# gmum/3d-point-clouds-autocomplete

Measured on AMD Instinct MI355X. Metric: train-step point-clouds/sec at B=64, N=2048 (Chamfer+EMD), higher is better.
Workload: dtype f32 storage / accumulation / results; matrix products formed from f16 x2 (bf16 x3) pieces of the fp32 operands — NOT IEEE-fp32 products: the all-fp32-kernel step is `value_strict_fp32`

## Files before the change

3d-point-clouds-autocomplete_amd/csrc/emd.hip:

```cpp
#include "hp_common.h"
#include <algorithm>
#include <map>
#include <mutex>
#include <vector>


namespace {

#ifndef HP_EMD_PARTS
#define HP_EMD_PARTS 4
#endif
constexpr int kThreads = 64 * HP_EMD_PARTS;
constexpr int kLevels = 9;
constexpr int kStage = 8;
constexpr int kSpare = 8;
constexpr float kLog2e = 1.4426950408889634f;

typedef float f32x16 __attribute__((ext_vector_type(16)));
typedef float f32x8 __attribute__((ext_vector_type(8)));
typedef float f2 __attribute__((ext_vector_type(2)));

#define HP_SLOAD16(dst, ptr, off) asm volatile("s_load_dwordx16 %0, %1, " #off : "=s"(dst) : "s"(ptr) : "memory")
#define HP_SLOAD8(dst, ptr, off) asm volatile("s_load_dwordx8 %0, %1, " #off : "=s"(dst) : "s"(ptr) : "memory")
#define HP_PIN() __builtin_amdgcn_sched_barrier(0)

__host__ __device__ constexpr float level_l2e(int lev) {
    return (lev == 0 ? -16384.f : lev == 1 ? -4096.f : lev == 2 ? -1024.f : lev == 3 ? -256.f : lev == 4 ? -64.f
            : lev == 5 ? -16.f : lev == 6 ? -4.f : lev == 7 ? -1.f : -0.25f) * kLog2e;
}
__host__ __device__ constexpr float underflow_r2(int lev) { return 152.f / -level_l2e(lev); }

constexpr int kParts = HP_EMD_PARTS;
constexpr int kRowsPerWg = kThreads / kParts;
inline int pad_up(int x) { return (x + 2 * kStage * kParts - 1) / (2 * kStage * kParts) * (2 * kStage * kParts); }

struct WsLayout {
    int NP, MP;
    long plp, prp, rr, flp, frp, permL, permR, blkL, blkR, tileL, tileR, flag, per_cloud;
};
constexpr int kBlk = 8;
constexpr int kTile = 64;
inline WsLayout ws_layout(int n, int m) {
    WsLayout w;
    w.NP = pad_up(n);
    w.MP = pad_up(m);
    w.plp = 0;
    w.prp = w.plp + (long)(w.NP + kSpare) * 4;
    w.rr = w.prp + (long)(w.MP + kSpare) * 4;
    w.flp = w.rr + (long)(w.MP + kSpare);
    w.frp = w.flp + (long)(w.NP + kSpare) * 16;
    w.permL = w.frp + (long)(w.MP + kSpare) * 16;
    w.permR = w.permL + w.NP;
    w.blkL = w.permR + w.MP;
    w.blkR = w.blkL + 6L * (w.NP / kBlk);
    w.tileL = w.blkR + 6L * (w.MP / kBlk);
    w.tileR = w.tileL + 6L * (w.NP / kTile);
    w.flag = w.tileR + 6L * (w.MP / kTile);
    w.per_cloud = w.flag + 16;
    return w;
}

std::mutex g_s2_mu;
std::map<int, hipStream_t> g_s2_streams;
constexpr int kMaxChains = 4;
constexpr int kOrderMaxLog = 12;
hp::Switch g_chains("HP_EMD_CHAINS", 2, 1, kMaxChains);
hp::Switch g_cull("HP_EMD_CULL", 3, 0, kLevels);
hp::Switch g_final_derive("HP_EMD_FINAL_DERIVE", 1);
hp::Switch g_rows1("HP_EMD_ROWS1_R", 0, 0, 4), g_rows2("HP_EMD_ROWS2_R", 0, 0, 4), g_grad2("HP_EMD_GRAD2_R", 0, 0, 2);
struct EmdSwitches {
    int chains, cull, rows1, rows2, grad2;
    bool derive;
};
EmdSwitches read_switches() {
    return {g_chains.get(), g_cull.get(), g_rows1.get(), g_rows2.get(), g_grad2.get(), g_final_derive.get() != 0};
}

struct Ctx {
    int n, m, NP, MP;
    const float* xyz1;
    const float* xyz2;
    float* temp;
    float* ws;
    int plp, prp, rr, flp, frp, permL, permR, blkL, blkR, tileL, tileR, flag;
    long per_cloud;
    float acc_scale = 0.f;
};
inline Ctx make_ctx(int n, int m, const float* xyz1, const float* xyz2, float* temp, float* ws) {
    const WsLayout L = ws_layout(n, m);
    Ctx c;
    c.n = n; c.m = m; c.NP = L.NP; c.MP = L.MP;
    c.xyz1 = xyz1; c.xyz2 = xyz2; c.temp = temp; c.ws = ws;
    c.plp = (int)L.plp; c.prp = (int)L.prp; c.rr = (int)L.rr; c.flp = (int)L.flp; c.frp = (int)L.frp;
    c.permL = (int)L.permL; c.permR = (int)L.permR; c.blkL = (int)L.blkL; c.blkR = (int)L.blkR; c.tileL = (int)L.tileL; c.tileR = (int)L.tileR;
    c.flag = (int)L.flag; c.per_cloud = L.per_cloud;
    c.acc_scale = 0.f;
    return c;
}

__device__ __forceinline__ long pair8(int i, int comp) { return (long)(i >> 1) * 8 + comp * 2 + (i & 1); }
__device__ __forceinline__ long pair32(int i, int comp) { return (long)(i >> 1) * 32 + comp * 2 + (i & 1); }

__global__ __launch_bounds__(256) void emd_init_kernel(Ctx c, float multiL, float multiR) {
    const int cloud = blockIdx.y;
    float* ws = c.ws + (long)cloud * c.per_cloud;
    float* remL = c.temp + (long)cloud * (c.n + c.m) * 2;
    float* remR = remL + c.n;
    const float* P = c.xyz1 + (long)cloud * c.n * 3;
    const float* Q = c.xyz2 + (long)cloud * c.m * 3;
    const int NPp = (c.NP + kSpare) / 2, MPp = (c.MP + kSpare) / 2;
    if (blockIdx.x == 0 && threadIdx.x == 0) ws[c.flag] = 0.f;
    for (int i = blockIdx.x * 256 + threadIdx.x; i < NPp + MPp; i += gridDim.x * 256) {
        const bool left = i < NPp;
        const int pr = left ? i : i - NPp, j0 = 2 * pr, j1 = j0 + 1;
        const int cnt = left ? c.n : c.m;
        const float* src = left ? P : Q;
        const bool ok0 = j0 < cnt, ok1 = j1 < cnt;
        const float x0 = ok0 ? src[j0 * 3] : 0.f, y0 = ok0 ? src[j0 * 3 + 1] : 0.f, z0 = ok0 ? src[j0 * 3 + 2] : 0.f;
        const float x1 = ok1 ? src[j1 * 3] : 0.f, y1 = ok1 ? src[j1 * 3 + 1] : 0.f, z1 = ok1 ? src[j1 * 3 + 2] : 0.f;
        float4* p8 = reinterpret_cast<float4*>(ws + (left ? c.plp : c.prp) + (long)pr * 8);
        float4* p32 = reinterpret_cast<float4*>(ws + (left ? c.flp : c.frp) + (long)pr * 32);
        const float4 a = make_float4(x0, x1, y0, y1), b = make_float4(z0, z1, 0.f, 0.f), zero = make_float4(0.f, 0.f, 0.f, 0.f);
        p8[0] = a;
        p8[1] = b;
        p32[0] = a;
        p32[1] = b;
#pragma unroll
        for (int q = 2; q < 8; ++q) p32[q] = zero;
        if (left) {
            if (ok0) remL[j0] = multiL;
            if (ok1) remL[j1] = multiL;
        } else {
            *reinterpret_cast<float2*>(ws + c.rr + j0) = make_float2(ok0 ? multiR : 0.f, ok1 ? multiR : 0.f);
            if (ok0) remR[j0] = multiR;
            if (ok1) remR[j1] = multiR;
        }
    }
}

// ... 176 lines not shown
    }
    const int NB = NPx / kBlk, NT = NPx / kTile;
    float* bb = ws + (left ? c.blkL : c.blkR);
    float* lb = box0;
    for (int g = tid; g < NB; g += kOrderThreads) {
        float lo[3] = {kFar, kFar, kFar}, hi[3] = {-kFar, -kFar, -kFar};
        for (int j = g * kBlk; j < min(g * kBlk + kBlk, cnt); ++j) {
            const uint32_t i = key[j] & imask;
            lo[0] = fminf(lo[0], X[i]); hi[0] = fmaxf(hi[0], X[i]);
            lo[1] = fminf(lo[1], Y[i]); hi[1] = fmaxf(hi[1], Y[i]);
            lo[2] = fminf(lo[2], Z[i]); hi[2] = fmaxf(hi[2], Z[i]);
        }
#pragma unroll
        for (int q = 0; q < 3; ++q) {
            bb[q * NB + g] = lo[q];
            bb[(3 + q) * NB + g] = hi[q];
            lb[g * 6 + q] = lo[q];
            lb[g * 6 + 3 + q] = hi[q];
        }
    }
    __syncthreads();
    float* tb = ws + (left ? c.tileL : c.tileR);
    for (int t = tid; t < NT; t += kOrderThreads) {
        float lo[3] = {kFar, kFar, kFar}, hi[3] = {-kFar, -kFar, -kFar};
        for (int g = t * (kTile / kBlk); g < (t + 1) * (kTile / kBlk); ++g) {
#pragma unroll
            for (int q = 0; q < 3; ++q) {
                lo[q] = fminf(lo[q], lb[g * 6 + q]);
                hi[q] = fmaxf(hi[q], lb[g * 6 + 3 + q]);
            }
        }
#pragma unroll
        for (int q = 0; q < 3; ++q) {
            tb[q * NT + t] = lo[q];
            tb[(3 + q) * NT + t] = hi[q];
        }
    }
    if (left && tid == 0) {
        ws[c.flag] = 1.f;
        ws[c.flag + 1] = cull > 1 ? underflow_r2(1) : 3.0e38f;
        ws[c.flag + 2] = cull > 2 ? underflow_r2(2) : 3.0e38f;
    }
}

#define PAIRC(lo, hi, u, c) \
    ((u) < 2 ? f2{(lo)[(u)*8 + (c)*2], (lo)[(u)*8 + (c)*2 + 1]} : f2{(hi)[((u)-2) * 8 + (c)*2], (hi)[((u)-2) * 8 + (c)*2 + 1]})

__device__ __forceinline__ f2 splat(float v) { return f2{v, v}; }
__device__ __forceinline__ f2 sqdist2(f2 dx, f2 dy, f2 dz) {
    return __builtin_elementwise_fma(dz, dz, __builtin_elementwise_fma(dy, dy, dx * dx));
}
__device__ __forceinline__ f2 exp2_2(f2 a) { return f2{__builtin_amdgcn_exp2f(a.x), __builtin_amdgcn_exp2f(a.y)}; }

template <bool DO3, bool DO1, int R>
__global__ __launch_bounds__(kThreads) void emd_rows1_kernel(Ctx c, int lev1, float l2e3, float l2e1) {
    __shared__ float part3[kParts][kRowsPerWg * R], part1[kParts][kRowsPerWg * R];
    const int cloud = blockIdx.y;
    const int lrow = threadIdx.x % kRowsPerWg;
    const int part = __builtin_amdgcn_readfirstlane(threadIdx.x / kRowsPerWg);
    float* ws = c.ws + (long)cloud * c.per_cloud;
    float* remL = c.temp + (long)cloud * (c.n + c.m) * 2;
    float* ratioL = remL + c.n + c.m;
    int k[R];
    bool ok[R];
    f2 px2[R], py2[R], pz2[R], rl2[R], acc3[R], acc1[R];
#pragma unroll
    for (int r = 0; r < R; ++r) {
        k[r] = (blockIdx.x * R + r) * kRowsPerWg + lrow;
        ok[r] = k[r] < c.n;
        float px = 0.f, py = 0.f, pz = 0.f, rl = 0.f;
        if (ok[r]) {
            px = ws[c.plp + pair8(k[r], 0)];
            py = ws[c.plp + pair8(k[r], 1)];
            pz = ws[c.plp + pair8(k[r], 2)];
            if (DO3) rl = ratioL[k[r]];
        }
        px2[r] = splat(px);
        py2[r] = splat(py);
        pz2[r] = splat(pz);
        rl2[r] = splat(rl);
        acc3[r] = splat(0.f);
        acc1[r] = f2{part == 0 ? 1e-9f : 0.f, 0.f};
    }
    const f2 l3 = splat(l2e3), l1 = splat(l2e1);
    const int cand = c.MP / kParts;
    const float* p = ws + c.prp + (long)part * cand * 4;
    const float* q = ws + c.rr + (long)part * cand;
    f32x16 a0, a1, b0, b1;
    f32x8 w0 = {}, w1 = {};
    auto work = [&](const f32x16& lo, const f32x16& hi, const f32x8& w) {
#pragma unroll
        for (int u = 0; u < kStage / 2; ++u) {
#pragma unroll
            for (int r = 0; r < R; ++r) {
                const f2 d = sqdist2(PAIRC(lo, hi, u, 0) - px2[r], PAIRC(lo, hi, u, 1) - py2[r], PAIRC(lo, hi, u, 2) - pz2[r]);
                if (DO3) {
                    acc3[r] = __builtin_elementwise_fma(exp2_2(l3 * d) * rl2[r], PAIRC(lo, hi, u, 3), acc3[r]);
                }
                if (DO1) {
                    acc1[r] = __builtin_elementwise_fma(exp2_2(l1 * d), f2{w[u * 2], w[u * 2 + 1]}, acc1[r]);
                }
            }
        }
    };
    HP_SLOAD16(a0, p, 0x0);
    HP_SLOAD16(a1, p, 0x40);
    if (DO1) HP_SLOAD8(w0, q, 0x0);
    asm volatile("s_waitcnt lgkmcnt(0)" : "+s"(a0), "+s"(a1), "+s"(w0));
    for (int l0 = 0; l0 < cand; l0 += 2 * kStage) {
        p += kStage * 4;
        q += kStage;
        HP_SLOAD16(b0, p, 0x0);
        HP_SLOAD16(b1, p, 0x40);
        if (DO1) HP_SLOAD8(w1, q, 0x0);
        HP_PIN();
        work(a0, a1, w0);
        asm volatile("s_waitcnt lgkmcnt(0)" : "+s"(b0), "+s"(b1), "+s"(w1), "+v"(acc3[0]), "+v"(acc1[0]), "+v"(acc3[R - 1]), "+v"(acc1[R - 1]));
        p += kStage * 4;
        q += kStage;
        HP_SLOAD16(a0, p, 0x0);
        HP_SLOAD16(a1, p, 0x40);
        if (DO1) HP_SLOAD8(w0, q, 0x0);
        HP_PIN();
        work(b0, b1, w1);
        asm volatile("s_waitcnt lgkmcnt(0)" : "+s"(a0), "+s"(a1), "+s"(w0), "+v"(acc3[0]), "+v"(acc1[0]), "+v"(acc3[R - 1]), "+v"(acc1[R - 1]));
    }
    float s3[R], s1[R];
#pragma unroll
    for (int r = 0; r < R; ++r) {
        s3[r] = acc3[r].x + acc3[r].y;
        s1[r] = acc1[r].x + acc1[r].y;
        part3[part][r * kRowsPerWg + lrow] = s3[r];
        part1[part][r * kRowsPerWg + lrow] = s1[r];
    }
    __syncthreads();
    if (part != 0) return;
#pragma unroll
    for (int r = 0; r < R; ++r) {
        if (!ok[r]) continue;
        float t3 = s3[r], t1 = s1[r];
#pragma unroll
        for (int q2 = 1; q2 < kParts; ++q2) {
            t3 += part3[q2][r * kRowsPerWg + lrow];
            t1 += part1[q2][r * kRowsPerWg + lrow];
        }
        float rem = remL[k[r]];
        if (DO3) {
            rem = fmaxf(0.0f, rem - t3);
            remL[k[r]] = rem;
        }
        if (DO1) {
            const float v = rem / t1;
            ratioL[k[r]] = v;
            ws[c.plp + pair8(k[r], 3)] = v;
            ws[c.flp + pair32(k[r], 3 + lev1)] = v;
        }
    }
}

template <int R>
__global__ __launch_bounds__(kThreads) void emd_rows2_kernel(Ctx c, int lev, float l2e) {
    __shared__ float parts[kParts][kRowsPerWg * R];
    const int cloud = blockIdx.y;
    const int lrow = threadIdx.x % kRowsPerWg;
    const int part = __builtin_amdgcn_readfirstlane(threadIdx.x / kRowsPerWg);
    float* ws = c.ws + (long)cloud * c.per_cloud;
    float* remR = c.temp + (long)cloud * (c.n + c.m) * 2 + c.n;
    float* ratioR = remR + c.m + c.n;
    int l[R];
    bool ok[R];
    f2 qx2[R], qy2[R], qz2[R], acc2[R];
#pragma unroll
    for (int r = 0; r < R; ++r) {
        l[r] = (blockIdx.x * R + r) * kRowsPerWg + lrow;
        ok[r] = l[r] < c.m;
        float qx = 0.f, qy = 0.f, qz = 0.f;
        if (ok[r]) {
            qx = ws[c.prp + pair8(l[r], 0)];
            qy = ws[c.prp + pair8(l[r], 1)];
            qz = ws[c.prp + pair8(l[r], 2)];
        }
        qx2[r] = splat(qx);
        qy2[r] = splat(qy);
        qz2[r] = splat(qz);
        acc2[r] = splat(0.f);
    }
    const f2 lv = splat(l2e);
    const int cand = c.NP / kParts;
    const float* p = ws + c.plp + (long)part * cand * 4;
    f32x16 a0, a1, b0, b1;
    auto work = [&](const f32x16& lo, const f32x16& hi) {
#pragma unroll
        for (int u = 0; u < kStage / 2; ++u) {
#pragma unroll
            for (int r = 0; r < R; ++r) {
                const f2 d = sqdist2(qx2[r] - PAIRC(lo, hi, u, 0), qy2[r] - PAIRC(lo, hi, u, 1), qz2[r] - PAIRC(lo, hi, u, 2));
                acc2[r] = __builtin_elementwise_fma(exp2_2(lv * d), PAIRC(lo, hi, u, 3), acc2[r]);
            }
        }
    };
    HP_SLOAD16(a0, p, 0x0);
    HP_SLOAD16(a1, p, 0x40);
    asm volatile("s_waitcnt lgkmcnt(0)" : "+s"(a0), "+s"(a1));
    for (int k0 = 0; k0 < cand; k0 += 2 * kStage) {
        p += kStage * 4;
        HP_SLOAD16(b0, p, 0x0);
        HP_SLOAD16(b1, p, 0x40);
        HP_PIN();
        work(a0, a1);
        if (R == 1) asm volatile("s_waitcnt lgkmcnt(0)" : "+s"(b0), "+s"(b1), "+v"(acc2[0]));
        else asm volatile("s_waitcnt lgkmcnt(0)" : "+s"(b0), "+s"(b1), "+v"(acc2[0]), "+v"(acc2[R - 1]));
        p += kStage * 4;
        HP_SLOAD16(a0, p, 0x0);
        HP_SLOAD16(a1, p, 0x40);
        HP_PIN();
        work(b0, b1);
        if (R == 1) asm volatile("s_waitcnt lgkmcnt(0)" : "+s"(a0), "+s"(a1), "+v"(acc2[0]));
        else asm volatile("s_waitcnt lgkmcnt(0)" : "+s"(a0), "+s"(a1), "+v"(acc2[0]), "+v"(acc2[R - 1]));
    }
    float acc[R];
#pragma unroll
    for (int r = 0; r < R; ++r) {
        acc[r] = acc2[r].x + acc2[r].y;
        parts[part][r * kRowsPerWg + lrow] = acc[r];
    }
    __syncthreads();
    if (part != 0) return;
#pragma unroll
    for (int r = 0; r < R; ++r) {
        if (!ok[r]) continue;
        float a = acc[r];
#pragma unroll
        for (int q2 = 1; q2 < kParts; ++q2) a += parts[q2][r * kRowsPerWg + lrow];
        const float rr = remR[l[r]];
        const float sumr = a * rr;
        const float consumption = fminf(rr / (sumr + 1e-9f), 1.0f);
        const float v = consumption * rr;
        const float rem = fmaxf(0.0f, rr - sumr);
        ratioR[l[r]] = v;
        remR[l[r]] = rem;
        ws[c.prp + pair8(l[r], 3)] = v;
        ws[c.rr + l[r]] = rem;
        ws[c.frp + pair32(l[r], 3 + lev)] = v;
    }
}

__device__ __forceinline__ float box_gap2(const float (&tlo)[3], const float (&thi)[3], float cx0, float cy0, float cz0, float cx1, float cy1,
                                          float cz1) {
    const float gx = fmaxf(0.f, fmaxf(cx0 - thi[0], tlo[0] - cx1));
    const float gy = fmaxf(0.f, fmaxf(cy0 - thi[1], tlo[1] - cy1));
    const float gz = fmaxf(0.f, fmaxf(cz0 - thi[2], tlo[2] - cz1));
    return gx * gx + gy * gy + gz * gz;
}
__device__ __forceinline__ void load_tile_box(const float* tb, int NT, int t, float (&lo)[3], float (&hi)[3]) {
#pragma unroll
    for (int q = 0; q < 3; ++q) {
        lo[q] = t < NT ? tb[q * NT + t] : kFar;
        hi[q] = t < NT ? tb[(3 + q) * NT + t] : -kFar;
    }
}

template <bool DO3, bool DO1, int R, int P>
__global__ __launch_bounds__(64 * P) void emd_rows1_cull_kernel(Ctx c, int lev1, float l2e3, float l2e1, float thr3, float thr1) {
    __shared__ float part3[P][kRowsPerWg * R], part1[P][kRowsPerWg * R];
    const int cloud = blockIdx.y;
    const int lrow = threadIdx.x % kRowsPerWg;
    const int part = __builtin_amdgcn_readfirstlane(threadIdx.x / kRowsPerWg);
    float* ws = c.ws + (long)cloud * c.per_cloud;
    float* remL = c.temp + (long)cloud * (c.n + c.m) * 2;
    float* ratioL = remL + c.n + c.m;
    int k[R];
    bool ok[R];
    f2 px2[R], py2[R], pz2[R], rl2[R], acc3[R], acc1[R];
    float tlo[R][3], thi[R][3];
#pragma unroll
    for (int r = 0; r < R; ++r) {
        k[r] = (blockIdx.x * R + r) * kRowsPerWg + lrow;
        ok[r] = k[r] < c.n;
        float px = 0.f, py = 0.f, pz = 0.f, rl = 0.f;
        if (ok[r]) {
            px = ws[c.plp + pair8(k[r], 0)];
            py = ws[c.plp + pair8(k[r], 1)];
            pz = ws[c.plp + pair8(k[r], 2)];
            if (DO3) rl = ratioL[k[r]];
        }
        px2[r] = splat(px);
        py2[r] = splat(py);
        pz2[r] = splat(pz);
        rl2[r] = splat(rl);
        acc3[r] = splat(0.f);
        acc1[r] = f2{part == 0 ? 1e-9f : 0.f, 0.f};
        load_tile_box(ws + c.tileL, c.NP / kTile, blockIdx.x * R + r, tlo[r], thi[r]);
    }
    const f2 l3 = splat(l2e3), l1 = splat(l2e1);
    const int NB = c.MP / kBlk, nblk = (NB + P - 1) / P;
    const float* bb = ws + c.blkR;
    const float* prec = ws + c.prp;
// ... 522 lines not shown
        parts[part][3][r * kRowsPerWg + lrow] = cost[r];
    }
    __syncthreads();
    float total = 0.f;
    if (part == 0) {
#pragma unroll
        for (int r = 0; r < R; ++r) {
#pragma unroll
            for (int q2 = 1; q2 < kParts; ++q2) {
                sx[r] += parts[q2][0][r * kRowsPerWg + lrow];
                sy[r] += parts[q2][1][r * kRowsPerWg + lrow];
                sz[r] += parts[q2][2][r * kRowsPerWg + lrow];
                cost[r] += parts[q2][3][r * kRowsPerWg + lrow];
            }
            if (ok[r]) {
                const int lo = ws[c.flag] != 0.f ? reinterpret_cast<const int*>(ws + c.permR)[l[r]] : l[r];
                float* g = grad2 + ((long)cloud * c.m + lo) * 3;
                if (c.acc_scale != 0.f) {
                    g[0] = __builtin_fmaf(c.acc_scale, sx[r], g[0]);
                    g[1] = __builtin_fmaf(c.acc_scale, sy[r], g[1]);
                    g[2] = __builtin_fmaf(c.acc_scale, sz[r], g[2]);
                } else {
                    g[0] = sx[r];
                    g[1] = sy[r];
                    g[2] = sz[r];
                }
                total += cost[r];
            }
        }
    }
    if (WITH_COST) {
        const float t = hp::block_sum(total, red);
        if (threadIdx.x == 0) partials[(long)cloud * gridDim.x + blockIdx.x] = t;
    }
}

__global__ __launch_bounds__(256) void emd_cost_finish_kernel(const float* __restrict__ partials, int per_cloud, float* __restrict__ out) {
    __shared__ double red[4];
    const float* p = partials + (long)blockIdx.x * per_cloud;
    double s = 0;
    for (int i = threadIdx.x; i < per_cloud; i += 256) s += (double)p[i];
    const double t = hp::block_sum(s, red);
    if (threadIdx.x == 0) out[blockIdx.x] = (float)t;
}

struct LevelChain {
    Ctx c;
    int b;
    hipStream_t stream;
    bool final_remainL;
    float multiL, multiR;
    int rows1_r, rows2_r;
    int cull;
    int logpL = 0, logpR = 0;
    dim3 ginit, g1[3], g2[3];

    static int log2_ceil64(int x) {
        int l = 6;
        while ((1 << l) < x) ++l;
        return l;
    }
    float radius2(int lev) const { return lev < cull ? underflow_r2(lev) : 3.0e38f; }

    LevelChain(int b_, int n, int m, const float* xyz1, const float* xyz2, float* temp, float* ws, hipStream_t st, bool frl,
               const EmdSwitches& sw)
        : b(b_), stream(st), final_remainL(frl), cull(sw.cull) {
        const WsLayout L = ws_layout(n, m);
        c = make_ctx(n, m, xyz1, xyz2, temp, ws);
        if (n >= m) {
            multiL = 1;
            multiR = (float)(n / m);
        } else {
            multiL = (float)(m / n);
            multiR = 1;
        }
        logpL = log2_ceil64(n);
        logpR = log2_ceil64(m);
        if (logpL > kOrderMaxLog || logpR > kOrderMaxLog) cull = 0;
        for (int i = 0; i < 3; ++i) {
            const int r = 1 << i;
            g1[i] = dim3((n + r * kRowsPerWg - 1) / (r * kRowsPerWg), b);
            g2[i] = dim3((m + r * kRowsPerWg - 1) / (r * kRowsPerWg), b);
        }
        ginit = dim3(((L.NP + L.MP + 2 * kSpare) / 2 + 255) / 256, b);
        auto pick = [&](int rows, int cap) {
            for (int r = cap; r > 1; r >>= 1)
                if ((long)b * ((rows + r * kRowsPerWg - 1) / (r * kRowsPerWg)) * (kThreads / 64) >= 2048) return r;
            return 1;
        };
        rows1_r = sw.rows1 ? sw.rows1 : pick(n, 2);
        rows2_r = sw.rows2 ? sw.rows2 : pick(m, 4);
    }

    template <bool D3, bool D1>
    void rows1(int lev3, int lev1) const {
        const float l2e3 = D3 ? level_l2e(lev3) : 0.f, l2e1 = D1 ? level_l2e(lev1) : 0.f;
        const int i = rows1_r == 4 ? 2 : rows1_r == 2 ? 1 : 0;
        const int clev = D1 ? lev1 : lev3;
        if (cull > 0 && clev < cull) {
            const float t3 = D3 ? radius2(lev3) : 0.f, t1 = D1 ? radius2(lev1) : 0.f;
            hipLaunchKernelGGL((emd_rows1_cull_kernel<D3, D1, 1, kParts>), g1[0], dim3(kThreads), 0, stream, c, lev1, l2e3, l2e1, t3, t1);
            return;
        }
        if (rows1_r == 4) hipLaunchKernelGGL((emd_rows1_kernel<D3, D1, 4>), g1[i], dim3(kThreads), 0, stream, c, lev1, l2e3, l2e1);
        else if (rows1_r == 2) hipLaunchKernelGGL((emd_rows1_kernel<D3, D1, 2>), g1[i], dim3(kThreads), 0, stream, c, lev1, l2e3, l2e1);
        else hipLaunchKernelGGL((emd_rows1_kernel<D3, D1, 1>), g1[i], dim3(kThreads), 0, stream, c, lev1, l2e3, l2e1);
    }
    void rows2(int lev) const {
        const int i = rows2_r == 4 ? 2 : rows2_r == 2 ? 1 : 0;
        if (cull > 0 && lev < cull) {
            const float t = radius2(lev);
            hipLaunchKernelGGL((emd_rows2_cull_kernel<1, kParts>), g2[0], dim3(kThreads), 0, stream, c, lev, level_l2e(lev), t);
            return;
        }
        if (rows2_r == 4) hipLaunchKernelGGL(emd_rows2_kernel<4>, g2[i], dim3(kThreads), 0, stream, c, lev, level_l2e(lev));
        else if (rows2_r == 2) hipLaunchKernelGGL(emd_rows2_kernel<2>, g2[i], dim3(kThreads), 0, stream, c, lev, level_l2e(lev));
        else hipLaunchKernelGGL(emd_rows2_kernel<1>, g2[i], dim3(kThreads), 0, stream, c, lev, level_l2e(lev));
    }
    static constexpr int kSteps = 2 + 2 * kLevels;
    void step(int s) const {
        if (s == 0) {
            if (cull > 0) {
                const int lp = std::max(logpL, logpR);
                const size_t lds = ((size_t)18 << lp) + kCells * 4;
                if (lds > 48 * 1024)
                    (void)hipFuncSetAttribute(reinterpret_cast<const void*>(emd_order_kernel), hipFuncAttributeMaxDynamicSharedMemorySize, (int)lds);
                hipLaunchKernelGGL(emd_order_kernel, dim3(2, b), dim3(kOrderThreads), lds, stream, c, multiL, multiR, logpL, logpR, cull);
            } else {
                hipLaunchKernelGGL(emd_init_kernel, ginit, dim3(256), 0, stream, c, multiL, multiR);
            }
        } else if (s == 1) {
            rows1<false, true>(0, 0);
        } else {
            const int lev = (s - 2) >> 1;
            if (((s - 2) & 1) == 0) rows2(lev);
            else if (lev + 1 < kLevels) rows1<true, true>(lev, lev + 1);
            else if (final_remainL) rows1<true, false>(lev, lev);
        }
    }
};

int run_levels(int b, int n, int m, const float* xyz1, const float* xyz2, float* temp, float* ws, Ctx* out, hipStream_t stream,
               bool final_remainL, const EmdSwitches& sw) {
    const LevelChain ch(b, n, m, xyz1, xyz2, temp, ws, stream, final_remainL, sw);
    for (int s = 0; s < LevelChain::kSteps; ++s) ch.step(s);
    *out = ch.c;
    return (int)hipGetLastError();
}

constexpr int kPlainTile = 1024;

__global__ __launch_bounds__(kThreads) void emd_plain_init_kernel(int n, int m, float* __restrict__ temp, float multiL, float multiR) {
    float* remL = temp + (long)blockIdx.y * (n + m) * 2;
    for (int i = blockIdx.x * kThreads + threadIdx.x; i < n + m; i += gridDim.x * kThreads) remL[i] = i < n ? multiL : multiR;
}

template <int PHASE>
__global__ __launch_bounds__(kThreads) void emd_plain_kernel(int n, int m, const float* __restrict__ xyz1, const float* __restrict__ xyz2,
                                                             float* __restrict__ temp, float* __restrict__ match, float l2e, int first) {
    __shared__ float4 tile[kPlainTile];
    const int cloud = blockIdx.y, tid = threadIdx.x;
    float* remL = temp + (long)cloud * (n + m) * 2;
    float* remR = remL + n;
    float* ratioL = remR + m;
    float* ratioR = ratioL + n;
    constexpr bool kRowsL = PHASE != 2;
    const int rows = kRowsL ? n : m, cands = kRowsL ? m : n;
    const float* R = (kRowsL ? xyz1 : xyz2) + (long)cloud * rows * 3;
    const float* C = (kRowsL ? xyz2 : xyz1) + (long)cloud * cands * 3;
    const float* cw = PHASE == 1 ? remR : PHASE == 2 ? ratioL : ratioR;
    const int row = blockIdx.x * kThreads + tid;
    const bool ok = row < rows;
    float rx = 0.f, ry = 0.f, rz = 0.f, rl = 0.f;
    if (ok) {
        rx = R[row * 3];
        ry = R[row * 3 + 1];
        rz = R[row * 3 + 2];
        if (PHASE == 3) rl = ratioL[row];
    }
    float sum = PHASE == 1 ? 1e-9f : 0.f;
    float* mcol = match + (long)cloud * m * n + row;
    for (int c0 = 0; c0 < cands; c0 += kPlainTile) {
        const int cnt = min(kPlainTile, cands - c0);
        for (int t = tid; t < cnt; t += kThreads) {
            const float* s = C + (long)(c0 + t) * 3;
            tile[t] = make_float4(s[0], s[1], s[2], cw[c0 + t]);
        }
        __syncthreads();
        if (ok) {
#pragma unroll 4
            for (int t = 0; t < cnt; ++t) {
                const float4 c = tile[t];
                const float d = kRowsL ? hp::sqdist(c.x - rx, c.y - ry, c.z - rz) : hp::sqdist(rx - c.x, ry - c.y, rz - c.z);
                const float e = __builtin_amdgcn_exp2f(l2e * d);
                if (PHASE == 3) {
                    const float er = e * rl;
                    float* mp = mcol + (long)(c0 + t) * n;
                    *mp = first ? er * c.w : __builtin_fmaf(er, c.w, *mp);
                    sum = __builtin_fmaf(er, c.w, sum);
                } else {
                    sum = __builtin_fmaf(e, c.w, sum);
                }
            }
        }
        __syncthreads();
    }
    if (!ok) return;
    if (PHASE == 1) {
        ratioL[row] = remL[row] / sum;
    } else if (PHASE == 2) {
        const float rr = remR[row];
        const float sumr = sum * rr;
        const float consumption = fminf(rr / (sumr + 1e-9f), 1.0f);
        ratioR[row] = consumption * rr;
        remR[row] = fmaxf(0.0f, rr - sumr);
    } else {
        remL[row] = fmaxf(0.0f, remL[row] - sum);
    }
}

}

HP_API int hp_emd_set_rows_per_lane(int rows1, int rows2, int grad2) {
    auto okv = [](int v, bool four) { return v == 0 || v == 1 || v == 2 || (four && v == 4); };
    HP_CHECK_ARG(okv(rows1, true) && okv(rows2, true) && okv(grad2, false));
    g_rows1.set(rows1);
    g_rows2.set(rows2);
    g_grad2.set(grad2);
    return 0;
}

HP_API int hp_emd_set_final_derive(int on) { return g_final_derive.set(on); }

HP_API int hp_emd_set_cull(int levels) {
    HP_CHECK_ARG(levels >= -1 && levels <= kLevels);
    return g_cull.set(levels);
}

HP_API int hp_emd_set_chains(int chains) {
    HP_CHECK_ARG(chains == -1 || (chains >= 1 && chains <= kMaxChains));
    return g_chains.set(chains);
}

HP_API int hp_approxmatch(int b, int n, int m, const float* xyz1, const float* xyz2, float* match, float* temp, hipStream_t stream) {
    HP_CHECK_ARG(b >= 0 && n > 0 && m > 0);
    if (b == 0) return 0;
    HP_CHECK_ARG(xyz1 && xyz2 && match && temp && b <= 65535);
    float multiL, multiR;
    if (n >= m) {
        multiL = 1;
        multiR = (float)(n / m);
    } else {
        multiL = (float)(m / n);
        multiR = 1;
    }
    const dim3 blk(kThreads), gL((n + kThreads - 1) / kThreads, b), gR((m + kThreads - 1) / kThreads, b);
    hipLaunchKernelGGL(emd_plain_init_kernel, dim3((n + m + kThreads - 1) / kThreads, b), blk, 0, stream, n, m, temp, multiL, multiR);
    for (int lev = 0; lev < kLevels; ++lev) {
        const float l2e = level_l2e(lev);
        hipLaunchKernelGGL(emd_plain_kernel<1>, gL, blk, 0, stream, n, m, xyz1, xyz2, temp, match, l2e, 0);
        hipLaunchKernelGGL(emd_plain_kernel<2>, gR, blk, 0, stream, n, m, xyz1, xyz2, temp, match, l2e, 0);
        hipLaunchKernelGGL(emd_plain_kernel<3>, gL, blk, 0, stream, n, m, xyz1, xyz2, temp, match, l2e, lev == 0);
    }
    HP_RETURN_LAST_ERROR();
}

HP_API long hp_approxmatch_workspace_floats(int b, int n, int m) { return (long)b * ws_layout(n, m).per_cloud; }

HP_API int hp_approxmatch_ws(int b, int n, int m, const float* xyz1, const float* xyz2, float* match, float* temp, float* ws,
                             hipStream_t stream) {
    HP_CHECK_ARG(b >= 0 && n > 0 && m > 0);
    if (b == 0) return 0;
    HP_CHECK_ARG(xyz1 && xyz2 && match && temp && ws && b <= 65535);
    Ctx c;
    EmdSwitches sw = read_switches();
    sw.cull = 0;
    int rc = run_levels(b, n, m, xyz1, xyz2, temp, ws, &c, stream, true, sw);
    if (rc) return rc;
    hipLaunchKernelGGL(emd_match_kernel, dim3((n + kThreads - 1) / kThreads, (m + kLT - 1) / kLT, b), dim3(kThreads), 0, stream, c,
                       match);
    HP_RETURN_LAST_ERROR();
}

HP_API long hp_emd_partials_floats(int b, int n, int m) { return (long)b * ((std::max(n, m) + kRowsPerWg - 1) / kRowsPerWg); }

namespace {
int emd_forward_impl(int b, int n, int m, const float* xyz1, const float* xyz2, float* temp, float* ws, float* partials,
                     float* cost, float* grad1, float* grad2, float acc_scale, hipStream_t stream, hipStream_t after);
}
HP_API int hp_emd_forward(int b, int n, int m, const float* xyz1, const float* xyz2, float* temp, float* ws, float* partials,
                          float* cost, float* grad1, float* grad2, hipStream_t stream) {
    return emd_forward_impl(b, n, m, xyz1, xyz2, temp, ws, partials, cost, grad1, grad2, 0.f, stream, nullptr);
}

HP_API int hp_emd_forward_acc(int b, int n, int m, const float* xyz1, const float* xyz2, float* temp, float* ws, float* partials,
                              float* cost, float* grad2_acc, float scale, hipStream_t stream, hipStream_t after) {
    HP_CHECK_ARG(grad2_acc && scale != 0.f);
    return emd_forward_impl(b, n, m, xyz1, xyz2, temp, ws, partials, cost, nullptr, grad2_acc, scale, stream, after);
}

namespace {
template <bool WITH_COST>
int launch_grad2(const Ctx& c, int b, float* grad2, float* partials, int rows, bool derive, hipStream_t stream) {
    const int mbr = (c.m + 2 * kRowsPerWg - 1) / (2 * kRowsPerWg);
    const bool two = (rows ? rows : ((long)b * mbr * (kThreads / 64) >= 2048 ? 2 : 1)) == 2;
    const dim3 grid(two ? mbr : (c.m + kRowsPerWg - 1) / kRowsPerWg, b);
    if (two) {
        if (derive) hipLaunchKernelGGL((emd_grad2_kernel<WITH_COST, 2, true>), grid, dim3(kThreads), 0, stream, c, grad2, partials);
        else hipLaunchKernelGGL((emd_grad2_kernel<WITH_COST, 2, false>), grid, dim3(kThreads), 0, stream, c, grad2, partials);
    } else {
        if (derive) hipLaunchKernelGGL((emd_grad2_kernel<WITH_COST, 1, true>), grid, dim3(kThreads), 0, stream, c, grad2, partials);
        else hipLaunchKernelGGL((emd_grad2_kernel<WITH_COST, 1, false>), grid, dim3(kThreads), 0, stream, c, grad2, partials);
    }
    return (int)grid.x;
}

int emd_final_sweep(Ctx c, int b, float* partials, float* cost, float* grad1, float* grad2, float acc_scale, hipStream_t stream,
                    hipStream_t after, const EmdSwitches& sw) {
    const int n = c.n;
    int rc = 0;
    c.acc_scale = acc_scale;
    if (after && after != stream) {
        rc = hp_order_streams(after, stream);
        if (rc) return rc;
    }
    const int nb = (n + kRowsPerWg - 1) / kRowsPerWg;
    if (grad2) {
        const int gb = launch_grad2<true>(c, b, grad2, partials, sw.grad2, sw.derive, stream);
        hipLaunchKernelGGL(emd_cost_finish_kernel, dim3(b), dim3(256), 0, stream, partials, gb, cost);
        if (grad1) {
            if (sw.derive) hipLaunchKernelGGL(emd_cost_grad1_kernel<true>, dim3(nb, b), dim3(kThreads), 0, stream, c, partials, grad1);
            else hipLaunchKernelGGL(emd_cost_grad1_kernel<false>, dim3(nb, b), dim3(kThreads), 0, stream, c, partials, grad1);
        }
    } else {
        if (sw.derive) hipLaunchKernelGGL(emd_cost_grad1_kernel<true>, dim3(nb, b), dim3(kThreads), 0, stream, c, partials, grad1);
        else hipLaunchKernelGGL(emd_cost_grad1_kernel<false>, dim3(nb, b), dim3(kThreads), 0, stream, c, partials, grad1);
        hipLaunchKernelGGL(emd_cost_finish_kernel, dim3(b), dim3(256), 0, stream, partials, nb, cost);
    }
    HP_RETURN_LAST_ERROR();
}


hipStream_t chain_stream(hipStream_t stream, int i) {
    int cur = 0, dev = 0;
    if (hipGetDevice(&cur) != hipSuccess) return nullptr;
    dev = cur;
    if (stream && hipStreamGetDevice(stream, &dev) != hipSuccess) {
        (void)hipGetLastError();
        dev = cur;
    }
    std::lock_guard<std::mutex> lock(g_s2_mu);
    auto it = g_s2_streams.find(dev * kMaxChains + i);
    if (it != g_s2_streams.end()) return it->second;
    hipStream_t s = nullptr;
    if (dev == cur || hipSetDevice(dev) == hipSuccess) {
        int lo = 0, hi = 0;
        (void)hipDeviceGetStreamPriorityRange(&lo, &hi);
        if (hipStreamCreateWithPriority(&s, hipStreamNonBlocking, hi) != hipSuccess) {
            (void)hipGetLastError();
            s = nullptr;
        }
        if (dev != cur) (void)hipSetDevice(cur);
    } else {
        (void)hipGetLastError();
    }
    g_s2_streams[dev * kMaxChains + i] = s;
    return s;
}

int emd_forward_impl(int b, int n, int m, const float* xyz1, const float* xyz2, float* temp, float* ws, float* partials,
                     float* cost, float* grad1, float* grad2, float acc_scale, hipStream_t stream, hipStream_t after) {
    HP_CHECK_ARG(b >= 0 && n > 0 && m > 0);
    if (b == 0) return 0;
    HP_CHECK_ARG(xyz1 && xyz2 && temp && ws && partials && cost && b <= 65535);
    const EmdSwitches sw = read_switches();
    hipStreamCaptureStatus cap = hipStreamCaptureStatusNone;
    (void)hipStreamIsCapturing(stream, &cap);
    int nch = cap == hipStreamCaptureStatusNone ? sw.chains : 1;
    while (nch > 1 && (long)(b / nch) * ((std::min(n, m) + kRowsPerWg - 1) / kRowsPerWg) * (kThreads / 64) < 2048) --nch;
    hipStream_t st[kMaxChains] = {stream};
    for (int i = 1; i < nch; ++i) {
        st[i] = chain_stream(stream, i);
        if (!st[i]) nch = 1;
    }
    if (nch <= 1) {
        Ctx c;
        const int rc = run_levels(b, n, m, xyz1, xyz2, temp, ws, &c, stream, false, sw);
        return rc ? rc : emd_final_sweep(c, b, partials, cost, grad1, grad2, acc_scale, stream, after, sw);
    }
    const WsLayout L = ws_layout(n, m);
    int rc = 0;
    for (int i = 1; i < nch && !rc; ++i) rc = hp_order_streams(stream, st[i]);
    if (rc) return rc;
    std::vector<LevelChain> ch;
    ch.reserve(nch);
    for (int i = 0; i < nch; ++i) {
        const int c0 = (int)((long)b * i / nch), c1 = (int)((long)b * (i + 1) / nch);
        ch.emplace_back(c1 - c0, n, m, xyz1 + (long)c0 * n * 3, xyz2 + (long)c0 * m * 3, temp + (long)c0 * (n + m) * 2, ws + (long)c0 * L.per_cloud,
                        st[i], false, sw);
    }
    for (int s = 0; s < LevelChain::kSteps; ++s)
        for (int i = 0; i < nch; ++i) ch[i].step(s);
    rc = (int)hipGetLastError();
    const bool ext = after && after != stream && acc_scale != 0.f;
    if (!rc && ext) rc = hp_order_streams(after, st[nch - 1]);
    for (int i = 1; i + 1 < nch; ++i) {
        const int r2 = hp_order_streams(st[i], st[i + 1]);
        if (!rc) rc = r2;
    }
    const int r3 = hp_order_streams(st[nch - 1], stream);
    if (!rc) rc = r3;
    if (rc) return rc;
    Ctx call = ch[0].c;
    return emd_final_sweep(call, b, partials, cost, grad1, grad2, acc_scale, stream, ext ? nullptr : after, sw);
}

}

HP_API int hp_emd_backward(int b, int n, int m, const float* xyz1, const float* xyz2, const float* ws, float* grad2,
                           hipStream_t stream) {
    HP_CHECK_ARG(b >= 0 && n > 0 && m > 0);
    if (b == 0) return 0;
    HP_CHECK_ARG(ws && grad2 && b <= 65535);
    const Ctx c = make_ctx(n, m, xyz1, xyz2, nullptr, const_cast<float*>(ws));
    launch_grad2<false>(c, b, grad2, nullptr, g_grad2.get(), g_final_derive.get() != 0, stream);
    HP_RETURN_LAST_ERROR();
}
```

include/hyperpocket_hip.h:

```cpp
#ifndef HYPERPOCKET_HIP_H
#define HYPERPOCKET_HIP_H

#ifdef __cplusplus
extern "C" {
#endif

typedef struct ihipStream_t* hpStream_t;


int hp_nndistance(int b, int n, const float* xyz, int m, const float* xyz2, float* result, int* result_i,
                  float* result2, int* result2_i, hpStream_t stream);

int hp_nndistancegrad(int b, int n, const float* xyz1, int m, const float* xyz2, const float* grad_dist1,
                      const int* idx1, const float* grad_dist2, const int* idx2, float* grad_xyz1, float* grad_xyz2,
                      hpStream_t stream);

int hp_approxmatch(int b, int n, int m, const float* xyz1, const float* xyz2, float* match, float* temp,
                   hpStream_t stream);
long hp_approxmatch_workspace_floats(int b, int n, int m);
int hp_approxmatch_ws(int b, int n, int m, const float* xyz1, const float* xyz2, float* match, float* temp, float* ws,
                      hpStream_t stream);
int hp_emd_set_rows_per_lane(int rows1, int rows2, int grad2);
int hp_emd_set_final_derive(int on);
int hp_emd_set_chains(int chains);
int hp_emd_set_cull(int levels);

long hp_emd_partials_floats(int b, int n, int m);
int hp_emd_forward(int b, int n, int m, const float* xyz1, const float* xyz2, float* temp, float* ws, float* partials,
                   float* cost, float* grad1 , float* grad2 , hpStream_t stream);
int hp_emd_forward_acc(int b, int n, int m, const float* xyz1, const float* xyz2, float* temp, float* ws, float* partials,
                       float* cost, float* grad2_acc, float scale, hpStream_t stream, hpStream_t after);
int hp_emd_backward(int b, int n, int m, const float* xyz1, const float* xyz2, const float* ws, float* grad2,
                    hpStream_t stream);

int hp_matchcost(int b, int n, int m, const float* xyz1, const float* xyz2, const float* match, float* out,
                 hpStream_t stream);
long hp_matchcost_workspace_floats(int b, int n, int m);
int hp_matchcost_ws(int b, int n, int m, const float* xyz1, const float* xyz2, const float* match, float* out,
                    float* partials, hpStream_t stream);

int hp_matchcostgrad(int b, int n, int m, const float* xyz1, const float* xyz2, const float* match, float* grad1,
                     float* grad2, hpStream_t stream);

long hp_chamfer_workspace_floats(int b, int n, int m);
int hp_chamfer_forward(int b, int n, const float* preds, int m, const float* gts, float* dist1, int* idx1,
                       float* dist2, int* idx2, float* partials, float* loss , hpStream_t stream);
int hp_chamfer_backward(int b, int n, const float* preds, int m, const float* gts, const int* idx1, const int* idx2,
                        const float* grad_loss , float* grad_preds, float* grad_gts,
                        hpStream_t stream);

#define HP_PAIRS_CHAMFER 0
#define HP_PAIRS_HAUSDORFF 1
#define HP_PAIRS_COVERED 2
long hp_cloud_pairs_workspace_floats(int mode, int n, int m, long pairs);
int hp_cloud_pairs(int mode, int na, int n, const float* A, int nb, int m, const float* B, long pairs,
                   const int* pair_ab, float thres, float* ws, float* out, hpStream_t stream);

#define HP_GEMM_BIAS 1
#define HP_GEMM_RELU 2
#define HP_GEMM_MASK 4
#define HP_GEMM_ADD 8
#define HP_GEMM_ROWSUM 32
#define HP_GEMM_COLMAX 16

typedef struct HpGemmDesc {
    const float* A;
    const float* B;
    float* C;
    const float* bias;
    const float* mask;
    const float* add;
    float* ws;
    long sAz, sBz, sCz, sBiasz, sMaskz, sAddz;
    long sAi, sAk, sBk, sBj;
    int ldc, ldmask, ldadd;
    int M, N, K, batch;
    int ksplit;
    int flags;
// ... 168 lines not shown
```

Before: 25270.

## Compact live EMD columns between levels to skip exhausted points

```diff
diff --git a/3d-point-clouds-autocomplete_amd/csrc/emd.hip b/3d-point-clouds-autocomplete_amd/csrc/emd.hip
--- a/3d-point-clouds-autocomplete_amd/csrc/emd.hip
+++ b/3d-point-clouds-autocomplete_amd/csrc/emd.hip
@@ -68,13 +68,31 @@
 hp::Switch g_cull("HP_EMD_CULL", 3, 0, kLevels);
 hp::Switch g_final_derive("HP_EMD_FINAL_DERIVE", 1);
 hp::Switch g_rows1("HP_EMD_ROWS1_R", 0, 0, 4), g_rows2("HP_EMD_ROWS2_R", 0, 0, 4), g_grad2("HP_EMD_GRAD2_R", 0, 0, 2);
+hp::Switch g_compact("HP_EMD_COMPACT", 1);
 struct EmdSwitches {
     int chains, cull, rows1, rows2, grad2;
-    bool derive;
+    bool derive, compact;
 };
 EmdSwitches read_switches() {
-    return {g_chains.get(), g_cull.get(), g_rows1.get(), g_rows2.get(), g_grad2.get(), g_final_derive.get() != 0};
-}
+    return {g_chains.get(), g_cull.get(), g_rows1.get(), g_rows2.get(), g_grad2.get(), g_final_derive.get() != 0, g_compact.get() != 0};
+}
+
+struct CsLayout {
+    long rec, w, list0, list1, cnt, per_cloud;
+};
+inline long align16(long x) { return (x + 15) / 16 * 16; }
+inline CsLayout cs_layout(int m) {
+    const int MP = pad_up(m);
+    CsLayout s;
+    s.rec = 0;
+    s.w = align16(s.rec + (long)(MP + kSpare) * 4);
+    s.list0 = align16(s.w + MP + kSpare);
+    s.list1 = align16(s.list0 + MP);
+    s.cnt = align16(s.list1 + MP);
+    s.per_cloud = align16(s.cnt + 16);
+    return s;
+}
+inline long cost_partials_floats(int b, int n, int m) { return align16((long)b * ((std::max(n, m) + kRowsPerWg - 1) / kRowsPerWg)); }
 
 struct Ctx {
     int n, m, NP, MP;
@@ -85,6 +103,8 @@
     int plp, prp, rr, flp, frp, permL, permR, blkL, blkR, tileL, tileR, flag;
     long per_cloud;
     float acc_scale = 0.f;
+    float* cs = nullptr;
+    int cs_rec = 0, cs_w = 0, cs_list0 = 0, cs_list1 = 0, cs_cnt = 0, cs_per_cloud = 0;
 };
 inline Ctx make_ctx(int n, int m, const float* xyz1, const float* xyz2, float* temp, float* ws) {
     const WsLayout L = ws_layout(n, m);
@@ -367,7 +387,7 @@
 }
 __device__ __forceinline__ f2 exp2_2(f2 a) { return f2{__builtin_amdgcn_exp2f(a.x), __builtin_amdgcn_exp2f(a.y)}; }
 
-template <bool DO3, bool DO1, int R>
+template <bool DO3, bool DO1, int R, bool COMPACT = false>
 __global__ __launch_bounds__(kThreads) void emd_rows1_kernel(Ctx c, int lev1, float l2e3, float l2e1) {
     __shared__ float part3[kParts][kRowsPerWg * R], part1[kParts][kRowsPerWg * R];
     const int cloud = blockIdx.y;
@@ -399,8 +419,10 @@
     }
     const f2 l3 = splat(l2e3), l1 = splat(l2e1);
     const int cand = c.MP / kParts;
-    const float* p = ws + c.prp + (long)part * cand * 4;
-    const float* q = ws + c.rr + (long)part * cand;
+    const float* cs = c.cs + (long)cloud * c.cs_per_cloud;
+    const float* p = (COMPACT ? cs + c.cs_rec : ws + c.prp) + (long)part * cand * 4;
+    const float* q = (COMPACT ? cs + c.cs_w : ws + c.rr) + (long)part * cand;
+    const int iters = COMPACT ? __builtin_amdgcn_readfirstlane(reinterpret_cast<const int*>(cs + c.cs_cnt)[4 + part]) : cand / (2 * kStage);
     f32x16 a0, a1, b0, b1;
     f32x8 w0 = {}, w1 = {};
     auto work = [&](const f32x16& lo, const f32x16& hi, const f32x8& w) {
@@ -422,7 +444,7 @@
     HP_SLOAD16(a1, p, 0x40);
     if (DO1) HP_SLOAD8(w0, q, 0x0);
     asm volatile("s_waitcnt lgkmcnt(0)" : "+s"(a0), "+s"(a1), "+s"(w0));
-    for (int l0 = 0; l0 < cand; l0 += 2 * kStage) {
+    for (int it = 0; it < iters; ++it) {
         p += kStage * 4;
         q += kStage;
         HP_SLOAD16(b0, p, 0x0);
@@ -473,8 +495,8 @@
     }
 }
 
-template <int R>
-__global__ __launch_bounds__(kThreads) void emd_rows2_kernel(Ctx c, int lev, float l2e) {
+template <int R, bool COMPACT = false>
+__global__ __launch_bounds__(kThreads) void emd_rows2_kernel(Ctx c, int lev, float l2e, int li) {
     __shared__ float parts[kParts][kRowsPerWg * R];
     const int cloud = blockIdx.y;
     const int lrow = threadIdx.x % kRowsPerWg;
@@ -482,13 +504,18 @@
     float* ws = c.ws + (long)cloud * c.per_cloud;
     float* remR = c.temp + (long)cloud * (c.n + c.m) * 2 + c.n;
     float* ratioR = remR + c.m + c.n;
+    const float* cs = c.cs + (long)cloud * c.cs_per_cloud;
+    const int* list = reinterpret_cast<const int*>(cs + (li ? c.cs_list1 : c.cs_list0));
+    const int rows = COMPACT ? __builtin_amdgcn_readfirstlane(reinterpret_cast<const int*>(cs + c.cs_cnt)[li]) : c.m;
+    if (COMPACT && (int)blockIdx.x * R * kRowsPerWg >= rows) return;
     int l[R];
     bool ok[R];
     f2 qx2[R], qy2[R], qz2[R], acc2[R];
 #pragma unroll
     for (int r = 0; r < R; ++r) {
-        l[r] = (blockIdx.x * R + r) * kRowsPerWg + lrow;
-        ok[r] = l[r] < c.m;
+        const int i = (blockIdx.x * R + r) * kRowsPerWg + lrow;
+        ok[r] = i < rows;
+        l[r] = COMPACT ? (ok[r] ? list[i] : 0) : i;
         float qx = 0.f, qy = 0.f, qz = 0.f;
         if (ok[r]) {
             qx = ws[c.prp + pair8(l[r], 0)];
@@ -558,6 +585,88 @@
         ws[c.rr + l[r]] = rem;
         ws[c.frp + pair32(l[r], 3 + lev)] = v;
     }
+}
+
+constexpr int kCompactThreads = 1024;
+constexpr int kClasses = 2 * kParts;
+
+__global__ __launch_bounds__(kCompactThreads) void emd_compact_kernel(Ctx c, int first, int li_in, int li_out) {
+    __shared__ int wtot[kCompactThreads / 64][kClasses + 1];
+    __shared__ int run[kClasses + 1];
+    const int tid = threadIdx.x, lane = tid & 63, wid = tid >> 6;
+    const int cloud = blockIdx.x;
+    const float* ws = c.ws + (long)cloud * c.per_cloud;
+    float* cs = c.cs + (long)cloud * c.cs_per_cloud;
+    float* ratioR = c.temp + (long)cloud * (c.n + c.m) * 2 + 2 * c.n + c.m;
+    int* cnt = reinterpret_cast<int*>(cs + c.cs_cnt);
+    const int* lin = reinterpret_cast<const int*>(cs + (li_in ? c.cs_list1 : c.cs_list0));
+    int* lout = reinterpret_cast<int*>(cs + (li_out ? c.cs_list1 : c.cs_list0));
+    float* rec = cs + c.cs_rec;
+    float* wr = cs + c.cs_w;
+    const int count = first ? c.m : cnt[li_in];
+    const int cand = c.MP / kParts;
+    const unsigned long long below = (1ull << lane) - 1ull;
+    if (tid <= kClasses) run[tid] = 0;
+    __syncthreads();
+    for (int base = 0; base < count; base += kCompactThreads) {
+        const int i = base + tid;
+        const bool valid = i < count;
+        const int l = valid ? (first ? i : lin[i]) : 0;
+        float x = 0.f, y = 0.f, z = 0.f, w = 0.f, rem = 0.f;
+        if (valid) {
+            x = ws[c.prp + pair8(l, 0)];
+            y = ws[c.prp + pair8(l, 1)];
+            z = ws[c.prp + pair8(l, 2)];
+            w = ws[c.prp + pair8(l, 3)];
+            rem = ws[c.rr + l];
+        }
+        const bool live = valid && rem != 0.f;
+        const bool keep = valid && (w != 0.f || rem != 0.f);
+        const int cls = (l / cand) * 2 + (l & 1);
+        const unsigned long long bl = __ballot(live);
+        if (lane == 0) wtot[wid][kClasses] = __popcll(bl);
+        int rank = 0;
+#pragma unroll
+        for (int q = 0; q < kClasses; ++q) {
+            const unsigned long long bq = __ballot(keep && cls == q);
+            if (cls == q) rank = __popcll(bq & below);
+            if (lane == 0) wtot[wid][q] = __popcll(bq);
+        }
+        __syncthreads();
+        int orow = run[kClasses] + __popcll(bl & below), ocls = run[cls] + rank;
+        for (int v = 0; v < wid; ++v) {
+            orow += wtot[v][kClasses];
+            ocls += wtot[v][cls];
+        }
+        if (live) lout[orow] = l;
+        else if (valid) ratioR[l] = 0.f;
+        if (keep) {
+            const int sl = (cls >> 1) * cand + 2 * ocls + (cls & 1);
+            rec[pair8(sl, 0)] = x;
+            rec[pair8(sl, 1)] = y;
+            rec[pair8(sl, 2)] = z;
+            rec[pair8(sl, 3)] = w;
+            wr[sl] = rem;
+        }
+        __syncthreads();
+        if (tid <= kClasses) {
+            int t = 0;
+            for (int v = 0; v < kCompactThreads / 64; ++v) t += wtot[v][tid];
+            run[tid] += t;
+        }
+        __syncthreads();
+    }
+    for (int sl = tid; sl < c.MP; sl += kCompactThreads) {
+        const int p = sl / cand, r = (sl - p * cand) >> 1, par = sl & 1;
+        const int end = (max(run[2 * p], run[2 * p + 1]) + kStage - 1) / kStage * kStage;
+        if (r >= run[2 * p + par] && r < end) {
+#pragma unroll
+            for (int q = 0; q < 4; ++q) rec[pair8(sl, q)] = 0.f;
+            wr[sl] = 0.f;
+        }
+    }
+    if (tid == 0) cnt[li_out] = run[kClasses];
+    if (tid < kParts) cnt[4 + tid] = (max(run[2 * tid], run[2 * tid + 1]) + kStage - 1) / kStage;
 }
 
 __device__ __forceinline__ float box_gap2(const float (&tlo)[3], const float (&thi)[3], float cx0, float cy0, float cz0, float cx1, float cy1,
@@ -1186,6 +1295,9 @@
     float multiL, multiR;
     int rows1_r, rows2_r;
     int cull;
+    bool compact = false;
+    int j0 = 0;
+    int rows2c_r = 1;
     int logpL = 0, logpR = 0;
     dim3 ginit, g1[3], g2[3];
 
@@ -1196,11 +1308,18 @@
     }
     float radius2(int lev) const { return lev < cull ? underflow_r2(lev) : 3.0e38f; }
 
-    LevelChain(int b_, int n, int m, const float* xyz1, const float* xyz2, float* temp, float* ws, hipStream_t st, bool frl,
+    LevelChain(int b_, int n, int m, const float* xyz1, const float* xyz2, float* temp, float* ws, float* cs, hipStream_t st, bool frl,
                const EmdSwitches& sw)
         : b(b_), stream(st), final_remainL(frl), cull(sw.cull) {
         const WsLayout L = ws_layout(n, m);
         c = make_ctx(n, m, xyz1, xyz2, temp, ws);
+        if (cs && sw.compact && !frl) {
+            const CsLayout S = cs_layout(m);
+            compact = true;
+            c.cs = cs;
+            c.cs_rec = (int)S.rec; c.cs_w = (int)S.w; c.cs_list0 = (int)S.list0; c.cs_list1 = (int)S.list1; c.cs_cnt = (int)S.cnt;
+            c.cs_per_cloud = (int)S.per_cloud;
+        }
         if (n >= m) {
             multiL = 1;
             multiR = (float)(n / m);
@@ -1224,6 +1343,8 @@
         };
         rows1_r = sw.rows1 ? sw.rows1 : pick(n, 2);
         rows2_r = sw.rows2 ? sw.rows2 : pick(m, 4);
+        rows2c_r = sw.rows2 ? sw.rows2 : pick(m, 2);
+        j0 = std::max(cull, 1) - 1;
     }
 
     template <bool D3, bool D1>
@@ -1236,6 +1357,12 @@
             hipLaunchKernelGGL((emd_rows1_cull_kernel<D3, D1, 1, kParts>), g1[0], dim3(kThreads), 0, stream, c, lev1, l2e3, l2e1, t3, t1);
             return;
         }
+        if (D3 && D1 && compact && lev3 >= j0) {
+            if (rows1_r == 4) hipLaunchKernelGGL((emd_rows1_kernel<true, true, 4, true>), g1[i], dim3(kThreads), 0, stream, c, lev1, l2e3, l2e1);
+            else if (rows1_r == 2) hipLaunchKernelGGL((emd_rows1_kernel<true, true, 2, true>), g1[i], dim3(kThreads), 0, stream, c, lev1, l2e3, l2e1);
+            else hipLaunchKernelGGL((emd_rows1_kernel<true, true, 1, true>), g1[i], dim3(kThreads), 0, stream, c, lev1, l2e3, l2e1);
+            return;
+        }
         if (rows1_r == 4) hipLaunchKernelGGL((emd_rows1_kernel<D3, D1, 4>), g1[i], dim3(kThreads), 0, stream, c, lev1, l2e3, l2e1);
         else if (rows1_r == 2) hipLaunchKernelGGL((emd_rows1_kernel<D3, D1, 2>), g1[i], dim3(kThreads), 0, stream, c, lev1, l2e3, l2e1);
         else hipLaunchKernelGGL((emd_rows1_kernel<D3, D1, 1>), g1[i], dim3(kThreads), 0, stream, c, lev1, l2e3, l2e1);
@@ -1247,9 +1374,20 @@
             hipLaunchKernelGGL((emd_rows2_cull_kernel<1, kParts>), g2[0], dim3(kThreads), 0, stream, c, lev, level_l2e(lev), t);
             return;
         }
-        if (rows2_r == 4) hipLaunchKernelGGL(emd_rows2_kernel<4>, g2[i], dim3(kThreads), 0, stream, c, lev, level_l2e(lev));
-        else if (rows2_r == 2) hipLaunchKernelGGL(emd_rows2_kernel<2>, g2[i], dim3(kThreads), 0, stream, c, lev, level_l2e(lev));
-        else hipLaunchKernelGGL(emd_rows2_kernel<1>, g2[i], dim3(kThreads), 0, stream, c, lev, level_l2e(lev));
+        if (compact && lev > j0) {
+            const int li = (lev - 1 - j0) & 1, ic = rows2c_r == 4 ? 2 : rows2c_r == 2 ? 1 : 0;
+            if (rows2c_r == 4) hipLaunchKernelGGL((emd_rows2_kernel<4, true>), g2[ic], dim3(kThreads), 0, stream, c, lev, level_l2e(lev), li);
+            else if (rows2c_r == 2) hipLaunchKernelGGL((emd_rows2_kernel<2, true>), g2[ic], dim3(kThreads), 0, stream, c, lev, level_l2e(lev), li);
+            else hipLaunchKernelGGL((emd_rows2_kernel<1, true>), g2[ic], dim3(kThreads), 0, stream, c, lev, level_l2e(lev), li);
+            return;
+        }
+        if (rows2_r == 4) hipLaunchKernelGGL(emd_rows2_kernel<4>, g2[i], dim3(kThreads), 0, stream, c, lev, level_l2e(lev), 0);
+        else if (rows2_r == 2) hipLaunchKernelGGL(emd_rows2_kernel<2>, g2[i], dim3(kThreads), 0, stream, c, lev, level_l2e(lev), 0);
+        else hipLaunchKernelGGL(emd_rows2_kernel<1>, g2[i], dim3(kThreads), 0, stream, c, lev, level_l2e(lev), 0);
+    }
+    void compact_after(int lev) const {
+        hipLaunchKernelGGL(emd_compact_kernel, dim3(b), dim3(kCompactThreads), 0, stream, c, lev == j0 ? 1 : 0, (lev - 1 - j0) & 1,
+                           (lev - j0) & 1);
     }
     static constexpr int kSteps = 2 + 2 * kLevels;
     void step(int s) const {
@@ -1267,16 +1405,18 @@
             rows1<false, true>(0, 0);
         } else {
             const int lev = (s - 2) >> 1;
-            if (((s - 2) & 1) == 0) rows2(lev);
-            else if (lev + 1 < kLevels) rows1<true, true>(lev, lev + 1);
+            if (((s - 2) & 1) == 0) {
+                rows2(lev);
+                if (compact && lev >= j0 && lev + 1 < kLevels) compact_after(lev);
+            } else if (lev + 1 < kLevels) rows1<true, true>(lev, lev + 1);
             else if (final_remainL) rows1<true, false>(lev, lev);
         }
     }
 };
 
-int run_levels(int b, int n, int m, const float* xyz1, const float* xyz2, float* temp, float* ws, Ctx* out, hipStream_t stream,
+int run_levels(int b, int n, int m, const float* xyz1, const float* xyz2, float* temp, float* ws, float* cs, Ctx* out, hipStream_t stream,
                bool final_remainL, const EmdSwitches& sw) {
-    const LevelChain ch(b, n, m, xyz1, xyz2, temp, ws, stream, final_remainL, sw);
+    const LevelChain ch(b, n, m, xyz1, xyz2, temp, ws, cs, stream, final_remainL, sw);
     for (int s = 0; s < LevelChain::kSteps; ++s) ch.step(s);
     *out = ch.c;
     return (int)hipGetLastError();
@@ -1371,6 +1511,8 @@
     return g_cull.set(levels);
 }
 
+HP_API int hp_emd_set_compact(int on) { return g_compact.set(on); }
+
 HP_API int hp_emd_set_chains(int chains) {
     HP_CHECK_ARG(chains == -1 || (chains >= 1 && chains <= kMaxChains));
     return g_chains.set(chains);
@@ -1409,14 +1551,14 @@
     Ctx c;
     EmdSwitches sw = read_switches();
     sw.cull = 0;
-    int rc = run_levels(b, n, m, xyz1, xyz2, temp, ws, &c, stream, true, sw);
+    int rc = run_levels(b, n, m, xyz1, xyz2, temp, ws, nullptr, &c, stream, true, sw);
     if (rc) return rc;
     hipLaunchKernelGGL(emd_match_kernel, dim3((n + kThreads - 1) / kThreads, (m + kLT - 1) / kLT, b), dim3(kThreads), 0, stream, c,
                        match);
     HP_RETURN_LAST_ERROR();
 }
 
-HP_API long hp_emd_partials_floats(int b, int n, int m) { return (long)b * ((std::max(n, m) + kRowsPerWg - 1) / kRowsPerWg); }
+HP_API long hp_emd_partials_floats(int b, int n, int m) { return cost_partials_floats(b, n, m) + (long)b * cs_layout(m).per_cloud; }
 
 namespace {
 int emd_forward_impl(int b, int n, int m, const float* xyz1, const float* xyz2, float* temp, float* ws, float* partials,
@@ -1517,9 +1659,11 @@
         st[i] = chain_stream(stream, i);
         if (!st[i]) nch = 1;
     }
+    float* cs = partials + cost_partials_floats(b, n, m);
+    const long cs_per_cloud = cs_layout(m).per_cloud;
     if (nch <= 1) {
         Ctx c;
-        const int rc = run_levels(b, n, m, xyz1, xyz2, temp, ws, &c, stream, false, sw);
+        const int rc = run_levels(b, n, m, xyz1, xyz2, temp, ws, cs, &c, stream, false, sw);
         return rc ? rc : emd_final_sweep(c, b, partials, cost, grad1, grad2, acc_scale, stream, after, sw);
     }
     const WsLayout L = ws_layout(n, m);
@@ -1531,7 +1675,7 @@
     for (int i = 0; i < nch; ++i) {
         const int c0 = (int)((long)b * i / nch), c1 = (int)((long)b * (i + 1) / nch);
         ch.emplace_back(c1 - c0, n, m, xyz1 + (long)c0 * n * 3, xyz2 + (long)c0 * m * 3, temp + (long)c0 * (n + m) * 2, ws + (long)c0 * L.per_cloud,
-                        st[i], false, sw);
+                        cs + c0 * cs_per_cloud, st[i], false, sw);
     }
     for (int s = 0; s < LevelChain::kSteps; ++s)
         for (int i = 0; i < nch; ++i) ch[i].step(s);
diff --git a/include/hyperpocket_hip.h b/include/hyperpocket_hip.h
--- a/include/hyperpocket_hip.h
+++ b/include/hyperpocket_hip.h
@@ -24,6 +24,7 @@
 int hp_emd_set_final_derive(int on);
 int hp_emd_set_chains(int chains);
 int hp_emd_set_cull(int levels);
+int hp_emd_set_compact(int on);
 
 long hp_emd_partials_floats(int b, int n, int m);
 int hp_emd_forward(int b, int n, int m, const float* xyz1, const float* xyz2, float* temp, float* ws, float* partials,
```

Result: faster. 27330 (median of 6 runs) (+8.1%).
